# tensorflow/lingvo

Hardware: AMD Instinct MI355X
Metric: train step examples/sec (whole node), Librispeech Conformer-L (higher is better)
Workload: dtype bf16; 1 GPU; model=Conformer-L (17 blocks, d=512, h=8, kernel 32) + LSTM attention decoder, global_batch=512, seq_len=1200, parallelism=dp1, step_mode=hipgraph

## Files before the change

lingvo_amd/ops/hip/bindings.cpp:

```cpp
#include <torch/extension.h>

#include <vector>

std::vector<torch::Tensor> layer_norm_fwd(torch::Tensor x,
                                          torch::Tensor scale,
                                          torch::Tensor bias, double eps,
                                          bool rms);
std::vector<torch::Tensor> layer_norm_bwd(torch::Tensor dy, torch::Tensor x,
                                          torch::Tensor scale,
                                          torch::Tensor mean,
                                          torch::Tensor rstd, bool rms,
                                          c10::optional<torch::Tensor> dres);

torch::Tensor mfma_probe(torch::Tensor a, torch::Tensor bT);
torch::Tensor tr16_probe(torch::Tensor a, torch::Tensor b);

std::vector<torch::Tensor> fa_fwd(torch::Tensor q, torch::Tensor k,
                                  torch::Tensor v,
                                  c10::optional<torch::Tensor> klen,
                                  c10::optional<torch::Tensor> bias,
                                  c10::optional<torch::Tensor> qseg,
                                  c10::optional<torch::Tensor> kseg,
                                  int64_t win_l, int64_t win_r,
                                  int64_t bias_clip, double scale,
// ... 31 lines not shown
std::vector<torch::Tensor> glu_dwconv1d_bwd(
    torch::Tensor dy, torch::Tensor h, c10::optional<torch::Tensor> paddings,
    torch::Tensor w, int64_t pad, const std::string& route,
    c10::optional<torch::Tensor> dh_out, c10::optional<torch::Tensor> dw_out,
    c10::optional<torch::Tensor> db_out,
    c10::optional<torch::Tensor> dcol_out);

int64_t dwconv_tile_len();

std::vector<torch::Tensor> xent_fwd(torch::Tensor logits,
                                    torch::Tensor labels);
torch::Tensor xent_bwd(torch::Tensor logits, torch::Tensor labels,
                       torch::Tensor lse, torch::Tensor gout);

torch::Tensor dropout_fwd(torch::Tensor x, c10::optional<torch::Tensor> res,
                          int64_t seed,
                          c10::optional<torch::Tensor> step_seed,
                          double keep, int64_t act, double scale,
                          c10::optional<torch::Tensor> pad, int64_t d);
torch::Tensor dropout_bwd(torch::Tensor dy, c10::optional<torch::Tensor> x,
                          int64_t seed,
                          c10::optional<torch::Tensor> step_seed,
                          double keep, int64_t act, double scale,
                          c10::optional<torch::Tensor> pad, int64_t d);
std::vector<torch::Tensor> dropout_bwd_colsum(
    torch::Tensor dy, c10::optional<torch::Tensor> x, int64_t seed,
    c10::optional<torch::Tensor> step_seed, double keep, int64_t act,
    double scale, c10::optional<torch::Tensor> pad, int64_t d);

std::vector<torch::Tensor> group_norm_fwd(torch::Tensor x,
                                          torch::Tensor gamma,
                                          torch::Tensor beta,
                                          c10::optional<torch::Tensor> pad,
                                          int64_t groups, double eps,
                                          int64_t act,
                                          const std::string& route);
std::vector<torch::Tensor> group_norm_bwd(torch::Tensor dy, torch::Tensor x,
                                          torch::Tensor gamma,
                                          torch::Tensor beta,
                                          c10::optional<torch::Tensor> pad,
                                          torch::Tensor mean,
                                          torch::Tensor rstd,
                                          int64_t groups, int64_t act);

std::vector<torch::Tensor> lstm_gates_fwd_op(torch::Tensor gates,
                                             torch::Tensor c0, double fgb,
                                             double cap);
std::vector<torch::Tensor> lstm_gates_bwd_op(
    torch::Tensor gates, torch::Tensor c0, torch::Tensor c1,
    torch::Tensor dm1, c10::optional<torch::Tensor> dc1, double fgb,
    double cap);

void RegisterInputPipeline(py::module_& m);

void RegisterWpmTokenizer(py::module_& m);

void RegisterRecordBatcher(py::module_& m);

torch::Tensor emb_gather(torch::Tensor table, torch::Tensor ids,
                         double scale);
torch::Tensor emb_scatter_add(torch::Tensor dy, torch::Tensor ids,
                              int64_t vocab, double scale);

std::vector<torch::Tensor> moe_positions(torch::Tensor top1,
                                         torch::Tensor top2,
                                         int64_t num_experts);

torch::Tensor s2d_fwd(torch::Tensor x);
torch::Tensor s2d_inv(torch::Tensor dX, int64_t C);
torch::Tensor pad_scatter(torch::Tensor dout);

std::vector<torch::Tensor> topk_rows(torch::Tensor scores, int64_t k);

void smallm_gemm(torch::Tensor a, torch::Tensor wt,
                 c10::optional<torch::Tensor> pre, torch::Tensor out,
                 int64_t k, int64_t wt_col0, double alpha,
                 int64_t pre_mode);
std::vector<torch::Tensor> attend_fwd(torch::Tensor q, torch::Tensor enc,
                                      torch::Tensor pad, double scale);
std::vector<torch::Tensor> attend_bwd(torch::Tensor dctx,
                                      torch::Tensor probs, torch::Tensor q,
                                      torch::Tensor enc, torch::Tensor denc,
                                      double scale);
int64_t attend_lds_limit();
int64_t attend_lds_bytes(int64_t s, int64_t d, bool bwd);

void lstm_scan_fwd(torch::Tensor gates, torch::Tensor c, torch::Tensor m,
                   torch::Tensor pad, torch::Tensor wmt, int64_t rev_mask,
                   double fgb, double cap, int64_t s_begin, int64_t s_end,
                   int64_t rows_per_block);
void lstm_scan_bwd(torch::Tensor gates, torch::Tensor c, torch::Tensor pad,
                   torch::Tensor wm, c10::optional<torch::Tensor> dm_out,
                   c10::optional<torch::Tensor> dc_out,
                   torch::Tensor dgates, torch::Tensor dc_carry,
                   torch::Tensor dm_pass, int64_t rev_mask, double fgb,
                   double cap, int64_t s_begin, int64_t s_end,
                   int64_t rows_per_block);

std::vector<torch::Tensor> ctc_fwd(torch::Tensor logits,
                                   torch::Tensor logit_lengths,
                                   torch::Tensor labels,
                                   torch::Tensor label_lengths,
                                   int64_t blank);
torch::Tensor ctc_bwd(torch::Tensor logits, torch::Tensor logit_lengths,
                      torch::Tensor labels, torch::Tensor label_lengths,
                      torch::Tensor lse, torch::Tensor emis,
                      torch::Tensor alpha, torch::Tensor beta,
                      torch::Tensor nll, torch::Tensor valid,
                      torch::Tensor gout, int64_t blank);
int64_t ctc_max_label_len();

std::vector<torch::Tensor> rnnt_fwd(torch::Tensor logits,
                                    torch::Tensor logit_lengths,
                                    torch::Tensor labels,
                                    torch::Tensor label_lengths,
                                    int64_t blank);
torch::Tensor rnnt_bwd(torch::Tensor logits, torch::Tensor logit_lengths,
                       torch::Tensor labels, torch::Tensor label_lengths,
                       torch::Tensor lse, torch::Tensor emis,
                       torch::Tensor alpha, torch::Tensor beta,
                       torch::Tensor valid, torch::Tensor gnll,
                       int64_t blank);
int64_t rnnt_max_label_len();

torch::Tensor attn_decode(torch::Tensor q, torch::Tensor key_cache,
                          torch::Tensor value_cache,
                          c10::optional<torch::Tensor> q_start_t,
                          int64_t q_start,
                          c10::optional<torch::Tensor> bias, int64_t win_l,
                          int64_t bias_clip, double scale,
                          int64_t num_splits);
int64_t attn_decode_num_splits(int64_t B, int64_t NKV, int64_t keys,
                               int64_t rows);

PYBIND11_MODULE(TORCH_EXTENSION_NAME, m) {
  RegisterInputPipeline(m);
  RegisterWpmTokenizer(m);
  RegisterRecordBatcher(m);
  m.def("group_norm_fwd", &group_norm_fwd, "Fused padded GroupNorm fwd",
        py::arg("x"), py::arg("gamma"), py::arg("beta"), py::arg("pad"),
        py::arg("groups"), py::arg("eps"), py::arg("act"),
        py::arg("route") = "auto");
  m.def("group_norm_bwd", &group_norm_bwd, "Fused padded GroupNorm bwd");
  m.def("lstm_gates_fwd", &lstm_gates_fwd_op, "Fused LSTM gates fwd");
  m.def("lstm_gates_bwd", &lstm_gates_bwd_op, "Fused LSTM gates bwd");
  m.def("dropout_fwd", &dropout_fwd, "Fused dropout fwd");
  m.def("dropout_bwd", &dropout_bwd, "Fused dropout bwd");
  m.def("dropout_bwd_colsum", &dropout_bwd_colsum,
        "Fused dropout bwd + fp32 column sums of dx");
  m.def("xent_fwd", &xent_fwd, "Fused softmax-xent fwd");
  m.def("xent_bwd", &xent_bwd, "Fused softmax-xent bwd");
  m.def("dwconv1d_fwd", &dwconv1d_fwd, "Depthwise time conv fwd",
        py::arg("x"), py::arg("w"), py::arg("bias"), py::arg("pad"),
        py::arg("route") = "auto", py::arg("y_out") = py::none());
  m.def("dwconv1d_bwd", &dwconv1d_bwd, "Depthwise time conv bwd",
        py::arg("dy"), py::arg("x"), py::arg("w"), py::arg("pad"),
        py::arg("route") = "auto", py::arg("dx_out") = py::none(),
        py::arg("dw_out") = py::none(), py::arg("db_out") = py::none());
  m.def("glu_dwconv1d_fwd", &glu_dwconv1d_fwd,
        "conv(mask * glu(h)) + bias in one kernel", py::arg("h"),
        py::arg("paddings"), py::arg("w"), py::arg("bias"), py::arg("pad"),
        py::arg("route") = "auto", py::arg("y_out") = py::none());
  m.def("glu_dwconv1d_bwd", &glu_dwconv1d_bwd,
        "dh, dw, db and the fp32 column sums of dh of glu_dwconv1d_fwd",
        py::arg("dy"), py::arg("h"), py::arg("paddings"), py::arg("w"),
        py::arg("pad"), py::arg("route") = "auto",
        py::arg("dh_out") = py::none(), py::arg("dw_out") = py::none(),
        py::arg("db_out") = py::none(), py::arg("dcol_out") = py::none());
  m.def("dwconv_tile_len", &dwconv_tile_len,
        "Time rows per tile of the tiled depthwise convolution");
  m.def("layer_norm_fwd", &layer_norm_fwd, "Fused LayerNorm/RMSNorm fwd");
  m.def("layer_norm_bwd", &layer_norm_bwd, "Fused LayerNorm/RMSNorm bwd",
        py::arg("dy"), py::arg("x"), py::arg("scale"), py::arg("mean"),
        py::arg("rstd"), py::arg("rms"), py::arg("dres") = py::none());
  m.def("mfma_probe", &mfma_probe, "MFMA 16x16x32 layout probe");
  m.def("tr16_probe", &tr16_probe, "ds_read_tr16_b64 layout probe");
  m.def("fa_fwd", &fa_fwd, "Flash attention forward");
  m.def("fa_bwd", &fa_bwd, "Flash attention backward", py::arg("dout"),
        py::arg("q"), py::arg("k"), py::arg("v"), py::arg("o"),
        py::arg("lse"), py::arg("klen"), py::arg("bias"), py::arg("qseg"),
        py::arg("kseg"), py::arg("bias_grad"), py::arg("win_l"),
        py::arg("win_r"), py::arg("bias_clip"), py::arg("scale"),
        py::arg("chunk_size"), py::arg("left_chunks"),
        py::arg("dq_out") = py::none(), py::arg("dk_out") = py::none(),
        py::arg("dv_out") = py::none(), py::arg("route") = "auto");
  m.def("emb_gather", &emb_gather, "Embedding gather fwd");
  m.def("emb_scatter_add", &emb_scatter_add,
        "Deterministic embedding scatter-add bwd");
  m.def("moe_positions", &moe_positions,
        "Deterministic MoE top-2 position scan");
  m.def("smallm_gemm", &smallm_gemm,
        "Small-M MFMA GEMM (decode-step projections)");
  m.def("attend_fwd", &attend_fwd, "Fused dot-attention step fwd");
  m.def("attend_bwd", &attend_bwd, "Fused dot-attention step bwd");
  m.def("attend_lds_limit", &attend_lds_limit,
        "Dynamic LDS bytes an attend_* launch may ask for on this device");
  m.def("attend_lds_bytes", &attend_lds_bytes,
        "Dynamic LDS bytes attend_fwd/attend_bwd ask for at (S, D)");
  m.def("lstm_scan_fwd", &lstm_scan_fwd,
        "Fused LSTM scan forward: one launch per step, all directions");
  m.def("lstm_scan_bwd", &lstm_scan_bwd,
        "Fused LSTM scan backward: one launch per step, all directions");
  m.def("ctc_fwd", &ctc_fwd,
        "CTC loss forward: nll, valid and the backward's workspaces");
  m.def("ctc_bwd", &ctc_bwd, "CTC loss backward: dlogits");
  m.def("ctc_max_label_len", &ctc_max_label_len,
        "Largest label width L the CTC kernels support");
  m.def("rnnt_fwd", &rnnt_fwd,
        "Transducer loss forward: nll, valid and the backward's workspaces");
  m.def("rnnt_bwd", &rnnt_bwd, "Transducer loss backward: dlogits");
  m.def("rnnt_max_label_len", &rnnt_max_label_len,
        "Largest label width U the transducer kernels support");
  m.def("attn_decode", &attn_decode,
        "KV-cache attention (ExtendStep/StreamStep): split-K decode kernel "
        "+ combine",
        py::arg("q"), py::arg("key_cache"), py::arg("value_cache"),
        py::arg("q_start_t"), py::arg("q_start"), py::arg("bias"),
        py::arg("win_l"), py::arg("bias_clip"), py::arg("scale"),
        py::arg("num_splits") = 0);
  m.def("attn_decode_num_splits", &attn_decode_num_splits,
        "Split count attn_decode picks for (B, NKV, keys, rows = C * N/NKV)",
        py::arg("B"), py::arg("NKV"), py::arg("keys"), py::arg("rows") = 1);
  m.def("s2d_fwd", &s2d_fwd, "Space-to-depth + pad (conv frontend)");
  m.def("topk_rows", &topk_rows, "Row-wise top-k (beam pruning, K12)");
  m.def("s2d_inv", &s2d_inv, "Inverse space-to-depth");
  m.def("pad_scatter", &pad_scatter, "Zero-border pad scatter");
}
```

lingvo_amd/ops/hip/las_decoder.hip:

```cpp

#include <torch/extension.h>
#include <ATen/hip/HIPContext.h>

#include <atomic>

#include "common.h"
#include "mfma.h"

namespace {

__global__ __launch_bounds__(256) void smallm_gemm_kernel(
    const unsigned short* __restrict__ a, const unsigned short* __restrict__ wt,
    const unsigned short* __restrict__ pre, unsigned short* __restrict__ out,
    int m, int n, int k, long ldw, float alpha, int pre_mode) {
  const int nt = blockIdx.x;
  const int col0 = nt * 16;
  const int m0 = blockIdx.y * 128;
  const int wid = threadIdx.x / WAVE_SIZE;
  const int lane = threadIdx.x & 63;
  const int g = lane >> 4;
  const int cl = lane & 15;
  const int col = col0 + cl;
  const bool col_ok = col < n;

  constexpr int MT = 8;
  __shared__ float red[3][128][16];

  const int kq = (k / 32 + 3) / 4 * 32;
  const int k_lo = wid * kq;
  const int k_hi = min(k, k_lo + kq);

  f32x4 acc[MT];
#pragma unroll
  for (int mt = 0; mt < MT; ++mt) acc[mt] = {0.f, 0.f, 0.f, 0.f};

  for (int k0 = k_lo; k0 < k_hi; k0 += 32) {
    bf16x8 bf;
    if (col_ok) {
      bf = load_bf16x8_bits(wt + (long)col * ldw + k0 + g * 8);
    } else {
      float z[8] = {0, 0, 0, 0, 0, 0, 0, 0};
      bf = pack_bf16x8(z);
    }
#pragma unroll
    for (int mt = 0; mt < MT; ++mt) {
      const int row = m0 + mt * 16 + cl;
      bf16x8 af;
      if (row < m) {
        af = load_bf16x8_bits(a + (long)row * k + k0 + g * 8);
      } else {
        float z[8] = {0, 0, 0, 0, 0, 0, 0, 0};
        af = pack_bf16x8(z);
      }
      acc[mt] = mfma16x16x32_bf16(af, bf, acc[mt]);
    }
  }

  if (wid > 0) {
#pragma unroll
    for (int mt = 0; mt < MT; ++mt) {
#pragma unroll
      for (int r = 0; r < 4; ++r) {
        red[wid - 1][mt * 16 + g * 4 + r][cl] = acc[mt][r];
      }
    }
  }
  __syncthreads();
  if (wid != 0) return;
#pragma unroll
  for (int mt = 0; mt < MT; ++mt) {
#pragma unroll
    for (int r = 0; r < 4; ++r) {
      const int lrow = mt * 16 + g * 4 + r;
      const int row = m0 + lrow;
      if (row >= m || !col_ok) continue;
      float v = (acc[mt][r] + red[0][lrow][cl] + red[1][lrow][cl] +
                 red[2][lrow][cl]) * alpha;
      long off = (long)row * n + col;
      if (pre_mode == 1) {
        v += bf16_bits_to_float(pre[col]);
      } else if (pre_mode == 2) {
        v += bf16_bits_to_float(pre[off]);
      } else if (pre_mode == 3) {
        v += bf16_bits_to_float(out[off]);
      }
      out[off] = float_to_bf16_bits(v);
    }
// ... 196 lines not shown
        float t = wave_reduce_sum(part[u]);
        if (lane == 0) dl_s[s0 + u] = t;
      }
    }
  }
  __syncthreads();
  float t_part = 0.f;
  for (int s = threadIdx.x; s < s_len; s += 256) {
    t_part += pb[s] * dl_s[s];
  }
  t_part = wave_reduce_sum(t_part);
  if (lane == 0) red[wid] = t_part;
  __syncthreads();
  const float t = red[0] + red[1] + red[2] + red[3];

  __syncthreads();
  for (int s = threadIdx.x; s < s_len; s += 256) {
    dl_s[s] = pb[s] * (dl_s[s] - t) * scale;
  }
  __syncthreads();

  for (int i = threadIdx.x; i < 4 * d; i += 256) dq_s[i] = 0.f;
  __syncthreads();
  float* my_dq = dq_s + wid * d;
  float* db = denc + (long)b * s_len * d;
  for (int s0 = wid * 4; s0 < s_len; s0 += 16) {
    float dlv[4], ppv[4];
#pragma unroll
    for (int u = 0; u < 4; ++u) {
      dlv[u] = s0 + u < s_len ? dl_s[s0 + u] : 0.f;
      ppv[u] = s0 + u < s_len ? pb[s0 + u] : 0.f;
    }
    for (int v = 0; v < ndv; ++v) {
      const int i = lane * 8 + v * WAVE_SIZE * 8;
      if (i < d) {
        bf16x8 ev[4];
        floatx4 lo[4], hi[4];
#pragma unroll
        for (int u = 0; u < 4; ++u) {
          if (s0 + u < s_len) {
            ev[u] = load_bf16x8_bits(eb + (long)(s0 + u) * d + i);
            floatx4* dbv =
                reinterpret_cast<floatx4*>(db + (long)(s0 + u) * d + i);
            lo[u] = dbv[0];
            hi[u] = dbv[1];
          }
        }
        float dqacc[8] = {0, 0, 0, 0, 0, 0, 0, 0};
#pragma unroll
        for (int u = 0; u < 4; ++u) {
          if (s0 + u < s_len) {
#pragma unroll
            for (int j = 0; j < 4; ++j) {
              dqacc[j] += dlv[u] * (float)ev[u][j];
              lo[u][j] += dlv[u] * qreg[v][j] + ppv[u] * dcreg[v][j];
            }
#pragma unroll
            for (int j = 4; j < 8; ++j) {
              dqacc[j] += dlv[u] * (float)ev[u][j];
              hi[u][j - 4] += dlv[u] * qreg[v][j] + ppv[u] * dcreg[v][j];
            }
          }
        }
#pragma unroll
        for (int u = 0; u < 4; ++u) {
          if (s0 + u < s_len) {
            floatx4* dbv =
                reinterpret_cast<floatx4*>(db + (long)(s0 + u) * d + i);
            dbv[0] = lo[u];
            dbv[1] = hi[u];
          }
        }
#pragma unroll
        for (int j = 0; j < 8; ++j) {
          my_dq[i + j] += dqacc[j];
        }
      }
    }
  }
  __syncthreads();
  for (int i = threadIdx.x; i < d; i += 256) {
    dq[(long)b * d + i] = float_to_bf16_bits(
        dq_s[i] + dq_s[d + i] + dq_s[2 * d + i] + dq_s[3 * d + i]);
  }
}

}


namespace {

size_t lds_limit_bytes() {
  constexpr int kMaxDevices = 64;
  static std::atomic<int> cached[kMaxDevices];
  int dev = 0;
  LV_CHECK_HIP(hipGetDevice(&dev));
  const bool cacheable = dev >= 0 && dev < kMaxDevices;
  int limit = cacheable ? cached[dev].load(std::memory_order_relaxed) : 0;
  if (limit == 0) {
    LV_CHECK_HIP(hipDeviceGetAttribute(
        &limit, hipDeviceAttributeMaxSharedMemoryPerBlock, dev));
    if (cacheable) cached[dev].store(limit, std::memory_order_relaxed);
  }
  return (size_t)limit;
}

constexpr int64_t kAttendMaxD = 4 * WAVE_SIZE * 8;

size_t attend_fwd_lds(int64_t s, int64_t d) {
  return (size_t)d * 2 + (size_t)s * 4 + (size_t)4 * d * 4 + 16;
}

size_t attend_bwd_lds(int64_t s, int64_t d) {
  return (size_t)d * 4 + (size_t)s * 4 + (size_t)4 * d * 4 + 16;
}

bool cuda_contig(const torch::Tensor& t, torch::ScalarType st) {
  return t.is_cuda() && t.is_contiguous() && t.scalar_type() == st;
}

void check_attend_q_enc(const torch::Tensor& q, const torch::Tensor& enc) {
  TORCH_CHECK(cuda_contig(q, torch::kBFloat16) && q.dim() == 2,
              "q must be CUDA contiguous bf16 [B,D]");
  TORCH_CHECK(cuda_contig(enc, torch::kBFloat16) && enc.dim() == 3,
              "enc must be CUDA contiguous bf16 [B,S,D]");
  const int64_t b = q.size(0), d = q.size(1);
  TORCH_CHECK(b >= 1 && enc.size(0) == b && enc.size(2) == d,
              "enc must be [B,S,D] for q [B,D]");
  TORCH_CHECK(enc.size(1) >= 1, "S >= 1");
  TORCH_CHECK(d >= 8 && d % 8 == 0, "D % 8 == 0");
  TORCH_CHECK(d <= kAttendMaxD, "D <= 2048");
}

}

void smallm_gemm(torch::Tensor a, torch::Tensor wt,
                 c10::optional<torch::Tensor> pre, torch::Tensor out,
                 int64_t k, int64_t wt_col0, double alpha,
                 int64_t pre_mode) {
  TORCH_CHECK(cuda_contig(a, torch::kBFloat16) && a.dim() == 2,
              "a must be CUDA contiguous bf16 [M,K]");
  TORCH_CHECK(cuda_contig(wt, torch::kBFloat16) && wt.dim() == 2,
              "wt must be CUDA contiguous bf16 [>=N,ldw]");
  TORCH_CHECK(cuda_contig(out, torch::kBFloat16) && out.dim() == 2,
              "out must be CUDA contiguous bf16 [M,N]");
  TORCH_CHECK(out.size(0) == a.size(0), "out must have M rows");
  const int m = a.size(0);
  const int n = out.size(1);
  TORCH_CHECK(m >= 1 && n >= 1, "M, N >= 1");
  TORCH_CHECK(k >= 32 && k % 32 == 0, "K%32");
  TORCH_CHECK(k == a.size(1), "a must be [M,K] exactly");

  TORCH_CHECK(wt.size(0) >= n, "wt rows >= N");
  const long ldw = wt.size(1);
  TORCH_CHECK(wt_col0 >= 0 && wt_col0 + k <= ldw, "wt K slice OOB");
  TORCH_CHECK(ldw % 8 == 0 && wt_col0 % 8 == 0,
              "ldw % 8 == 0 and wt_col0 % 8 == 0");
  TORCH_CHECK(pre_mode >= 0 && pre_mode <= 3, "pre_mode in 0..3");
  const unsigned short* prep = nullptr;
  if (pre_mode == 1 || pre_mode == 2) {
    TORCH_CHECK(pre.has_value() && cuda_contig(*pre, torch::kBFloat16),
                "pre must be CUDA contiguous bf16");
    if (pre_mode == 1) {
      TORCH_CHECK(pre->numel() == n, "mode 1: pre must have N elements");
    } else {
      TORCH_CHECK(pre->dim() == 2 && pre->size(0) == m && pre->size(1) == n,
                  "mode 2: pre must be [M,N]");
    }
    prep = (const unsigned short*)pre->data_ptr();
  }
  auto stream = at::cuda::getCurrentCUDAStream();
  hipLaunchKernelGGL(smallm_gemm_kernel,
                     dim3(cdiv(n, 16), cdiv(m, 128)), dim3(256), 0,
                     stream, (const unsigned short*)a.data_ptr(),
                     (const unsigned short*)wt.data_ptr() + wt_col0,
                     prep, (unsigned short*)out.data_ptr(), m, n, (int)k,
                     ldw, (float)alpha, (int)pre_mode);
  LV_CHECK_HIP(hipGetLastError());
}

std::vector<torch::Tensor> attend_fwd(torch::Tensor q, torch::Tensor enc,
                                      torch::Tensor pad, double scale) {
  check_attend_q_enc(q, enc);
  const int b = q.size(0), d = q.size(1);
  const int s = enc.size(1);
  TORCH_CHECK(cuda_contig(pad, torch::kFloat32) && pad.dim() == 2 &&
              pad.size(0) == b && pad.size(1) == s,
              "pad must be CUDA contiguous fp32 [B,S]");
  const size_t shmem = attend_fwd_lds(s, d);
  TORCH_CHECK(shmem <= lds_limit_bytes(), "attend_fwd: S=", s, " D=", d,
              " needs ", shmem, " bytes of LDS, over the device limit");
  auto probs = torch::empty({b, s}, q.options().dtype(torch::kFloat32));
  auto ctx = torch::empty({b, d}, q.options());
  auto stream = at::cuda::getCurrentCUDAStream();
  hipLaunchKernelGGL(attend_fwd_kernel, dim3(b), dim3(256), shmem, stream,
                     (const unsigned short*)q.data_ptr(),
                     (const unsigned short*)enc.data_ptr(),
                     pad.data_ptr<float>(), probs.data_ptr<float>(),
                     (unsigned short*)ctx.data_ptr(), b, s, d,
                     (float)scale);
  LV_CHECK_HIP(hipGetLastError());
  return {probs, ctx};
}

std::vector<torch::Tensor> attend_bwd(torch::Tensor dctx,
                                      torch::Tensor probs, torch::Tensor q,
                                      torch::Tensor enc, torch::Tensor denc,
                                      double scale) {
  check_attend_q_enc(q, enc);
  const int b = q.size(0), d = q.size(1);
  const int s = enc.size(1);
  TORCH_CHECK(dctx.is_cuda() && dctx.is_floating_point() &&
              dctx.dim() == 2 && dctx.size(0) == b && dctx.size(1) == d,
              "dctx must be a CUDA float tensor [B,D]");
  TORCH_CHECK(cuda_contig(probs, torch::kFloat32) && probs.dim() == 2 &&
              probs.size(0) == b && probs.size(1) == s,
              "probs must be CUDA contiguous fp32 [B,S]");
  TORCH_CHECK(cuda_contig(denc, torch::kFloat32) && denc.dim() == 3 &&
              denc.size(0) == b && denc.size(1) == s && denc.size(2) == d,
              "denc must be CUDA contiguous fp32 [B,S,D]");
  const size_t shmem = attend_bwd_lds(s, d);
  TORCH_CHECK(shmem <= lds_limit_bytes(), "attend_bwd: S=", s, " D=", d,
              " needs ", shmem, " bytes of LDS, over the device limit");
  auto dctx_c = dctx.to(torch::kBFloat16).contiguous();
  auto dq = torch::empty({b, d}, q.options());
  auto stream = at::cuda::getCurrentCUDAStream();
  hipLaunchKernelGGL(attend_bwd_kernel, dim3(b), dim3(256), shmem, stream,
                     (const unsigned short*)dctx_c.data_ptr(),
                     probs.data_ptr<float>(),
                     (const unsigned short*)q.data_ptr(),
                     (const unsigned short*)enc.data_ptr(),
                     (unsigned short*)dq.data_ptr(),
                     denc.data_ptr<float>(), b, s, d, (float)scale);
  LV_CHECK_HIP(hipGetLastError());
  return {dq};
}

int64_t attend_lds_limit() { return (int64_t)lds_limit_bytes(); }

int64_t attend_lds_bytes(int64_t s, int64_t d, bool bwd) {
  return (int64_t)(bwd ? attend_bwd_lds(s, d) : attend_fwd_lds(s, d));
}
```

lingvo_amd/ops/las_decoder.py:

```python

from __future__ import annotations

import math
from typing import Optional

import torch

from lingvo_amd.ops import _loader


class _DecoderRecurrenceFn(torch.autograd.Function):

  @staticmethod
  def forward(ctx, emb_gates, w_cm0, b1, wm1, wq, enc, enc_pad, fgb, cap,
              src_dim):
    ext = _loader.get_ext(required=True)
    B, L, G4 = emb_gates.shape
    H = G4 // 4
    D = wq.shape[1]
    scale = 1.0 / math.sqrt(D)
    dt = torch.bfloat16
    emb_gates_b = emb_gates.to(dt).contiguous()
    enc_b = enc.to(dt).contiguous()
    pad_f = enc_pad.float().contiguous()
    w1t = w_cm0.t().contiguous().to(dt)
    wm1t = wm1.t().contiguous().to(dt)
    wqt = wq.t().contiguous().to(dt)
    b1_b = b1.to(dt).contiguous()

    dev = enc.device
    gates0 = torch.empty(L, B, G4, dtype=dt, device=dev)
    gates1 = torch.empty(L, B, G4, dtype=dt, device=dev)
    qs = torch.empty(L, B, D, dtype=dt, device=dev)
    eg_t = emb_gates_b.permute(1, 0, 2).contiguous()
    c0s, m0s, c1s, m1s, ctxs, probs_l = [], [], [], [], [], []
    zeros_h = torch.zeros(B, H, dtype=dt, device=dev)
    c0, m0, c1, m1 = zeros_h, zeros_h, zeros_h, zeros_h
    ctxv = torch.zeros(B, D, dtype=dt, device=dev)
    for t in range(L):
      g0 = gates0[t]
      ext.smallm_gemm(ctxv, w1t, eg_t[t], g0, src_dim, 0, 1.0, 2)
      ext.smallm_gemm(m0, w1t, None, g0, H, src_dim, 1.0, 3)
      c0, m0 = ext.lstm_gates_fwd(g0, c0, fgb, cap)
      g1 = gates1[t]
      ext.smallm_gemm(m0, wm1t, b1_b, g1, H, 0, 1.0, 1)
      ext.smallm_gemm(m1, wm1t, None, g1, H, H, 1.0, 3)
      c1, m1 = ext.lstm_gates_fwd(g1, c1, fgb, cap)
      q = qs[t]
      ext.smallm_gemm(m1, wqt, None, q, H, 0, 1.0, 0)
      p, ctxv = ext.attend_fwd(q, enc_b, pad_f, scale)
      c0s.append(c0)
      m0s.append(m0)
      c1s.append(c1)
      m1s.append(m1)
      ctxs.append(ctxv)
      probs_l.append(p)

    m1_st = torch.stack(m1s)
    ctx_st = torch.stack(ctxs)
    ctx.save_for_backward(
        emb_gates_b, w_cm0, wm1, wq, enc_b, pad_f, gates0, gates1, qs,
        torch.stack(c0s), torch.stack(m0s), torch.stack(c1s), m1_st,
        ctx_st, torch.stack(probs_l))
    ctx.cfg = (fgb, cap, src_dim, scale, b1.dtype, enc.dtype,
               emb_gates.dtype)
    out = torch.cat(
        [m1_st.permute(1, 0, 2), ctx_st.permute(1, 0, 2)], dim=-1)
    return out

  @staticmethod
  def backward(ctx, dout):
    ext = _loader.get_ext(required=True)
    (emb_gates_b, w_cm0, wm1, wq, enc_b, pad_f, gates0, gates1, qs, c0s,
     m0s, c1s, m1s, ctxs, probs) = ctx.saved_tensors
    fgb, cap, src_dim, scale, b1_dtype, enc_dtype, eg_dtype = ctx.cfg
    L, B, G4 = gates0.shape
    H = G4 // 4
    D = qs.shape[-1]
    dt = torch.bfloat16
    dev = dout.device
    dout = dout.to(dt)
    w_cm0_b = w_cm0.to(dt).contiguous()
    wm1_b = wm1.to(dt).contiguous()
    wq_b = wq.to(dt).contiguous()

    denc = torch.zeros(B, enc_b.shape[1], D, dtype=torch.float32,
                       device=dev)
    dgates0 = torch.empty(L, B, G4, dtype=dt, device=dev)
    dgates1 = torch.empty(L, B, G4, dtype=dt, device=dev)
    dqs = torch.empty(L, B, D, dtype=dt, device=dev)
    zeros_h = torch.zeros(B, H, dtype=dt, device=dev)
    dctx_carry = torch.zeros(B, D, dtype=dt, device=dev)
    dm0_carry = zeros_h
    dm1_carry = zeros_h
    dc0_carry: Optional[torch.Tensor] = None
    dc1_carry: Optional[torch.Tensor] = None
    dmm = torch.empty(B, 2 * H, dtype=dt, device=dev)
    dcm = torch.empty(B, src_dim + H, dtype=dt, device=dev)
    dm1_total = torch.empty(B, H, dtype=dt, device=dev)
    dout_t = dout.permute(1, 0, 2)
    dm1_parts = dout_t[:, :, :H].contiguous()
    dctx_parts = dout_t[:, :, H:].contiguous()
    for t in range(L - 1, -1, -1):
      dctx_total = dctx_parts[t] + dctx_carry
      dq = ext.attend_bwd(dctx_total, probs[t], qs[t], enc_b, denc,
                          scale)[0]
      dqs[t] = dq
      pre_m1 = dm1_parts[t] + dm1_carry
      ext.smallm_gemm(dq, wq_b, pre_m1, dm1_total, D, 0, 1.0, 2)
      c1_prev = c1s[t - 1] if t > 0 else zeros_h
      dg1, dc1_carry = ext.lstm_gates_bwd(
          gates1[t], c1_prev, c1s[t], dm1_total, dc1_carry, fgb, cap)
      dgates1[t] = dg1
      ext.smallm_gemm(dg1, wm1_b, None, dmm, G4, 0, 1.0, 0)
      dm0_total = (dmm[:, :H] + dm0_carry).contiguous()
      c0_prev = c0s[t - 1] if t > 0 else zeros_h
      dg0, dc0_carry = ext.lstm_gates_bwd(
          gates0[t], c0_prev, c0s[t], dm0_total, dc0_carry, fgb, cap)
      dgates0[t] = dg0
      ext.smallm_gemm(dg0, w_cm0_b, None, dcm, G4, 0, 1.0, 0)
      dctx_carry = dcm[:, :src_dim].contiguous()
      dm0_carry = dcm[:, src_dim:].contiguous()
      dm1_carry = dmm[:, H:].contiguous()

    ctx_prev = torch.cat(
        [torch.zeros(1, B, D, dtype=dt, device=dev), ctxs[:-1]])
    m0_prev = torch.cat(
        [torch.zeros(1, B, H, dtype=dt, device=dev), m0s[:-1]])
    m1_prev = torch.cat(
        [torch.zeros(1, B, H, dtype=dt, device=dev), m1s[:-1]])
    x0 = torch.cat([ctx_prev, m0_prev], dim=-1).reshape(L * B, -1)
    dw_cm0 = (x0.t() @ dgates0.reshape(L * B, G4)).to(w_cm0.dtype)
    x1 = torch.cat([m0s, m1_prev], dim=-1).reshape(L * B, -1)
    dwm1 = (x1.t() @ dgates1.reshape(L * B, G4)).to(wm1.dtype)
    db1 = dgates1.float().sum(dim=(0, 1)).to(b1_dtype)
    dwq = (m1s.reshape(L * B, H).t() @ dqs.reshape(L * B, D)).to(wq.dtype)
    demb_gates = dgates0.permute(1, 0, 2).to(eg_dtype)
    return (demb_gates, dw_cm0, db1, dwm1, dwq, denc.to(enc_dtype),
            None, None, None, None)


def decoder_recurrence(emb_gates: torch.Tensor, w_cm0: torch.Tensor,
                       b1: torch.Tensor, wm1: torch.Tensor,
                       wq: torch.Tensor, enc: torch.Tensor,
                       enc_pad: torch.Tensor, fgb: float, cap: float,
                       src_dim: int) -> torch.Tensor:
  return _DecoderRecurrenceFn.apply(emb_gates, w_cm0, b1, wm1, wq, enc,
                                    enc_pad, fgb, cap, src_dim)
```

Measured before the change: 1399 examples/sec.

## Defer decoder attention dEnc to one batched kernel after the recurrence

Adds one-pass attention step kernels. The forward writes probs, ctx and an fp32 ctx into preallocated stacked buffers. The backward now emits only dctx, dlogits and dq per step and no longer accumulates dEnc into a [B,S,D] fp32 buffer at every decoder step. The encoder gradient is then computed once after the loop by a tiled kernel that sums over all steps, as dl·q + p·dctx. This removes the per-step read-modify-write of the full dEnc tensor, at the cost of storing per-step dl, dctx and ctx32 stacks. It is enabled by default through the 'auto' route.

```diff
diff --git a/lingvo_amd/ops/hip/bindings.cpp b/lingvo_amd/ops/hip/bindings.cpp
--- a/lingvo_amd/ops/hip/bindings.cpp
+++ b/lingvo_amd/ops/hip/bindings.cpp
@@ -137,6 +137,18 @@
                                       torch::Tensor probs, torch::Tensor q,
                                       torch::Tensor enc, torch::Tensor denc,
                                       double scale);
+void attend_step_fwd(torch::Tensor q, torch::Tensor enc, torch::Tensor pad,
+                     double scale, torch::Tensor probs, torch::Tensor ctx,
+                     torch::Tensor ctx32, int64_t variant);
+void attend_step_bwd(torch::Tensor dctx_a, c10::optional<torch::Tensor> dctx_b,
+                     torch::Tensor probs, torch::Tensor ctx32,
+                     torch::Tensor enc, double scale, torch::Tensor dctx_out,
+                     torch::Tensor dl, torch::Tensor dq, int64_t variant);
+void attend_denc(torch::Tensor dl, torch::Tensor probs, torch::Tensor qs,
+                 torch::Tensor dctx, torch::Tensor out);
+int64_t attend_step_lds_bytes(int64_t s, int64_t d, bool bwd,
+                              int64_t variant);
+int64_t attend_denc_row_tile();
 int64_t attend_lds_limit();
 int64_t attend_lds_bytes(int64_t s, int64_t d, bool bwd);
 
@@ -248,6 +260,23 @@
         "Small-M MFMA GEMM (decode-step projections)");
   m.def("attend_fwd", &attend_fwd, "Fused dot-attention step fwd");
   m.def("attend_bwd", &attend_bwd, "Fused dot-attention step bwd");
+  m.def("attend_step_fwd", &attend_step_fwd,
+        "One-pass dot-attention step fwd into caller rows (probs, ctx, ctx32)",
+        py::arg("q"), py::arg("enc"), py::arg("pad"), py::arg("scale"),
+        py::arg("probs"), py::arg("ctx"), py::arg("ctx32"),
+        py::arg("variant") = 0);
+  m.def("attend_step_bwd", &attend_step_bwd,
+        "One-pass dot-attention step bwd without dEnc (dctx, dl, dq out)",
+        py::arg("dctx_a"), py::arg("dctx_b"), py::arg("probs"),
+        py::arg("ctx32"), py::arg("enc"), py::arg("scale"),
+        py::arg("dctx_out"), py::arg("dl"), py::arg("dq"),
+        py::arg("variant") = 0);
+  m.def("attend_denc", &attend_denc,
+        "dEnc of the whole recurrence from the stacked dl, probs, q, dctx");
+  m.def("attend_step_lds_bytes", &attend_step_lds_bytes,
+        "Dynamic LDS bytes attend_step_fwd/bwd ask for at (S, D, variant)");
+  m.def("attend_denc_row_tile", &attend_denc_row_tile,
+        "Rows of S one attend_denc workgroup owns");
   m.def("attend_lds_limit", &attend_lds_limit,
         "Dynamic LDS bytes an attend_* launch may ask for on this device");
   m.def("attend_lds_bytes", &attend_lds_bytes,
diff --git a/lingvo_amd/ops/hip/las_decoder.hip b/lingvo_amd/ops/hip/las_decoder.hip
--- a/lingvo_amd/ops/hip/las_decoder.hip
+++ b/lingvo_amd/ops/hip/las_decoder.hip
@@ -3,6 +3,7 @@
 #include <ATen/hip/HIPContext.h>
 
 #include <atomic>
+#include <climits>
 
 #include "common.h"
 #include "mfma.h"
@@ -365,6 +366,312 @@
   for (int i = threadIdx.x; i < d; i += 256) {
     dq[(long)b * d + i] = float_to_bf16_bits(
         dq_s[i] + dq_s[d + i] + dq_s[2 * d + i] + dq_s[3 * d + i]);
+  }
+}
+
+
+
+template <int NDV, int U>
+__device__ __forceinline__ void load_enc_rows(
+    const unsigned short* __restrict__ eb, int s0, int s_len, int d, int lane,
+    bf16x8 (&ev)[U][NDV]) {
+  const float z[8] = {0, 0, 0, 0, 0, 0, 0, 0};
+  const bf16x8 zero = pack_bf16x8(z);
+#pragma unroll
+  for (int u = 0; u < U; ++u) {
+#pragma unroll
+    for (int v = 0; v < NDV; ++v) {
+      const int i = lane * 8 + v * WAVE_SIZE * 8;
+      ev[u][v] = (s0 + u < s_len && i < d)
+                     ? load_bf16x8_bits(eb + (long)(s0 + u) * d + i)
+                     : zero;
+    }
+  }
+}
+
+template <int NDV, int U, int NW>
+__global__ __launch_bounds__(NW * WAVE_SIZE) void attend_step_fwd_kernel(
+    const unsigned short* __restrict__ q, const unsigned short* __restrict__ enc,
+    const float* __restrict__ pad, float* __restrict__ probs,
+    unsigned short* __restrict__ ctx, float* __restrict__ ctx32, int s_len,
+    int d, float scale) {
+  constexpr int NT = NW * WAVE_SIZE;
+  const int b = blockIdx.x;
+  const int wid = threadIdx.x / WAVE_SIZE;
+  const int lane = threadIdx.x & 63;
+  extern __shared__ char smem[];
+  float* logit_s = (float*)smem;
+  float* ctx_s = logit_s + s_len;
+  float* red = ctx_s + NW * d;
+
+  float qreg[NDV][8];
+#pragma unroll
+  for (int v = 0; v < NDV; ++v) {
+    const int i = lane * 8 + v * WAVE_SIZE * 8;
+    if (i < d) {
+      bf16x8 qv = load_bf16x8_bits(q + (long)b * d + i);
+#pragma unroll
+      for (int j = 0; j < 8; ++j) qreg[v][j] = (float)qv[j];
+    } else {
+#pragma unroll
+      for (int j = 0; j < 8; ++j) qreg[v][j] = 0.f;
+    }
+  }
+
+  const unsigned short* eb = enc + (long)b * s_len * d;
+  const float* padb = pad + (long)b * s_len;
+  float m = -1e30f;
+  float acc[NDV][8];
+#pragma unroll
+  for (int v = 0; v < NDV; ++v) {
+#pragma unroll
+    for (int j = 0; j < 8; ++j) acc[v][j] = 0.f;
+  }
+  for (int s0 = wid * U; s0 < s_len; s0 += NW * U) {
+    bf16x8 ev[U][NDV];
+    load_enc_rows<NDV, U>(eb, s0, s_len, d, lane, ev);
+    float mask[U];
+#pragma unroll
+    for (int u = 0; u < U; ++u) {
+      mask[u] = (s0 + u >= s_len || padb[s0 + u] > 0.5f) ? -1e30f : 0.f;
+    }
+    float lg[U];
+    float mnew = m;
+#pragma unroll
+    for (int u = 0; u < U; ++u) {
+      float part = 0.f;
+#pragma unroll
+      for (int v = 0; v < NDV; ++v) {
+#pragma unroll
+        for (int j = 0; j < 8; ++j) part += qreg[v][j] * (float)ev[u][v][j];
+      }
+      lg[u] = wave_reduce_sum(part) * scale + mask[u];
+      if (s0 + u < s_len) {
+        mnew = fmaxf(mnew, lg[u]);
+        if (lane == 0) logit_s[s0 + u] = lg[u];
+      }
+    }
+    const float f = __expf(m - mnew);
+    m = mnew;
+#pragma unroll
+    for (int v = 0; v < NDV; ++v) {
+#pragma unroll
+      for (int j = 0; j < 8; ++j) acc[v][j] *= f;
+    }
+#pragma unroll
+    for (int u = 0; u < U; ++u) {
+      const float p = __expf(lg[u] - mnew);
+#pragma unroll
+      for (int v = 0; v < NDV; ++v) {
+#pragma unroll
+        for (int j = 0; j < 8; ++j) acc[v][j] += p * (float)ev[u][v][j];
+      }
+    }
+  }
+  if (lane == 0) red[wid] = m;
+  __syncthreads();
+  float lmax = red[0];
+#pragma unroll
+  for (int w = 1; w < NW; ++w) lmax = fmaxf(lmax, red[w]);
+  {
+    const float wgt = __expf(m - lmax);
+#pragma unroll
+    for (int v = 0; v < NDV; ++v) {
+      const int i = lane * 8 + v * WAVE_SIZE * 8;
+      if (i < d) {
+#pragma unroll
+        for (int j = 0; j < 8; ++j) ctx_s[wid * d + i + j] = acc[v][j] * wgt;
+      }
+    }
+  }
+  float lsum = 0.f;
+  for (int s = threadIdx.x; s < s_len; s += NT) {
+    float e = __expf(logit_s[s] - lmax);
+    logit_s[s] = e;
+    lsum += e;
+  }
+  lsum = wave_reduce_sum(lsum);
+  __syncthreads();
+  if (lane == 0) red[wid] = lsum;
+  __syncthreads();
+  lsum = 0.f;
+#pragma unroll
+  for (int w = 0; w < NW; ++w) lsum += red[w];
+  const float inv = lsum > 0.f ? 1.f / lsum : 0.f;
+  for (int s = threadIdx.x; s < s_len; s += NT) {
+    probs[(long)b * s_len + s] = logit_s[s] * inv;
+  }
+  for (int i = threadIdx.x; i < d; i += NT) {
+    float c = 0.f;
+#pragma unroll
+    for (int w = 0; w < NW; ++w) c += ctx_s[w * d + i];
+    c *= inv;
+    ctx32[(long)b * d + i] = c;
+    ctx[(long)b * d + i] = float_to_bf16_bits(c);
+  }
+}
+
+template <int NDV, int U, int NW>
+__global__ __launch_bounds__(NW * WAVE_SIZE) void attend_step_bwd_kernel(
+    const unsigned short* __restrict__ dctx_a,
+    const unsigned short* __restrict__ dctx_b, long ldb,
+    const float* __restrict__ probs, const float* __restrict__ ctx32,
+    const unsigned short* __restrict__ enc,
+    unsigned short* __restrict__ dctx_out, float* __restrict__ dl_out,
+    unsigned short* __restrict__ dq, int s_len, int d, float scale) {
+  constexpr int NT = NW * WAVE_SIZE;
+  const int b = blockIdx.x;
+  const int wid = threadIdx.x / WAVE_SIZE;
+  const int lane = threadIdx.x & 63;
+  extern __shared__ char smem[];
+  float* dc_s = (float*)smem;
+  float* dq_s = dc_s + d;
+  float* red = dq_s + NW * d;
+
+  float t_part = 0.f;
+  for (int i = threadIdx.x; i < d; i += NT) {
+    unsigned short bits = dctx_a[(long)b * d + i];
+    if (dctx_b != nullptr) {
+      bits = float_to_bf16_bits(bf16_bits_to_float(bits) +
+                                bf16_bits_to_float(dctx_b[(long)b * ldb + i]));
+    }
+    dctx_out[(long)b * d + i] = bits;
+    const float v = bf16_bits_to_float(bits);
+    dc_s[i] = v;
+    t_part += v * ctx32[(long)b * d + i];
+  }
+  const float t = block_reduce_sum<NW>(t_part, red);
+
+  float dcreg[NDV][8];
+#pragma unroll
+  for (int v = 0; v < NDV; ++v) {
+    const int i = lane * 8 + v * WAVE_SIZE * 8;
+#pragma unroll
+    for (int j = 0; j < 8; ++j) dcreg[v][j] = i < d ? dc_s[i + j] : 0.f;
+  }
+
+  const unsigned short* eb = enc + (long)b * s_len * d;
+  const float* pb = probs + (long)b * s_len;
+  float* dlb = dl_out + (long)b * s_len;
+  float acc[NDV][8];
+#pragma unroll
+  for (int v = 0; v < NDV; ++v) {
+#pragma unroll
+    for (int j = 0; j < 8; ++j) acc[v][j] = 0.f;
+  }
+  for (int s0 = wid * U; s0 < s_len; s0 += NW * U) {
+    bf16x8 ev[U][NDV];
+    load_enc_rows<NDV, U>(eb, s0, s_len, d, lane, ev);
+    float pv[U];
+#pragma unroll
+    for (int u = 0; u < U; ++u) pv[u] = s0 + u < s_len ? pb[s0 + u] : 0.f;
+#pragma unroll
+    for (int u = 0; u < U; ++u) {
+      float part = 0.f;
+#pragma unroll
+      for (int v = 0; v < NDV; ++v) {
+#pragma unroll
+        for (int j = 0; j < 8; ++j) part += dcreg[v][j] * (float)ev[u][v][j];
+      }
+      const float dlv = pv[u] * (wave_reduce_sum(part) - t) * scale;
+      if (lane == u && s0 + u < s_len) dlb[s0 + u] = dlv;
+#pragma unroll
+      for (int v = 0; v < NDV; ++v) {
+#pragma unroll
+        for (int j = 0; j < 8; ++j) acc[v][j] += dlv * (float)ev[u][v][j];
+      }
+    }
+  }
+#pragma unroll
+  for (int v = 0; v < NDV; ++v) {
+    const int i = lane * 8 + v * WAVE_SIZE * 8;
+    if (i < d) {
+#pragma unroll
+      for (int j = 0; j < 8; ++j) dq_s[wid * d + i + j] = acc[v][j];
+    }
+  }
+  __syncthreads();
+  for (int i = threadIdx.x; i < d; i += NT) {
+    float c = 0.f;
+#pragma unroll
+    for (int w = 0; w < NW; ++w) c += dq_s[w * d + i];
+    dq[(long)b * d + i] = float_to_bf16_bits(c);
+  }
+}
+
+constexpr int kDencRows = 8;
+constexpr int kDencTile = 4 * kDencRows;
+constexpr int kDencSteps = 64;
+
+__device__ __forceinline__ void store_denc(float* p, const float* a) {
+  floatx4* pv = reinterpret_cast<floatx4*>(p);
+  pv[0] = floatx4{a[0], a[1], a[2], a[3]};
+  pv[1] = floatx4{a[4], a[5], a[6], a[7]};
+}
+
+__device__ __forceinline__ void store_denc(unsigned short* p, const float* a) {
+  ushortx8 o;
+#pragma unroll
+  for (int j = 0; j < 8; ++j) o[j] = float_to_bf16_bits(a[j]);
+  *reinterpret_cast<ushortx8*>(p) = o;
+}
+
+template <typename OutT>
+__global__ __launch_bounds__(256) void attend_denc_kernel(
+    const float* __restrict__ dl, const float* __restrict__ probs,
+    const unsigned short* __restrict__ qs,
+    const unsigned short* __restrict__ dctx, OutT* __restrict__ out,
+    int l_total, int b_total, int s_len, int d, int s_tiles) {
+  const int b = blockIdx.x / s_tiles;
+  const int s_base = (blockIdx.x % s_tiles) * kDencTile;
+  const int wid = threadIdx.x / WAVE_SIZE;
+  const int lane = threadIdx.x & 63;
+  const int c0 = blockIdx.y * WAVE_SIZE * 8 + lane * 8;
+  __shared__ float sc[kDencSteps][kDencTile][2];
+
+  float acc[kDencRows][8];
+#pragma unroll
+  for (int r = 0; r < kDencRows; ++r) {
+#pragma unroll
+    for (int j = 0; j < 8; ++j) acc[r][j] = 0.f;
+  }
+  for (int l0 = 0; l0 < l_total; l0 += kDencSteps) {
+    __syncthreads();
+    for (int idx = threadIdx.x; idx < kDencSteps * kDencTile; idx += 256) {
+      const int ll = idx / kDencTile, r = idx % kDencTile;
+      const int l = l0 + ll, s = s_base + r;
+      const bool ok = l < l_total && s < s_len;
+      const long off = ((long)l * b_total + b) * s_len + s;
+      sc[ll][r][0] = ok ? dl[off] : 0.f;
+      sc[ll][r][1] = ok ? probs[off] : 0.f;
+    }
+    __syncthreads();
+    if (c0 < d) {
+      const int l_cnt = min(kDencSteps, l_total - l0);
+#pragma unroll 4
+      for (int ll = 0; ll < l_cnt; ++ll) {
+        const long off = ((long)(l0 + ll) * b_total + b) * d + c0;
+        const bf16x8 qv = load_bf16x8_bits(qs + off);
+        const bf16x8 dv = load_bf16x8_bits(dctx + off);
+#pragma unroll
+        for (int r = 0; r < kDencRows; ++r) {
+          const float a = sc[ll][wid * kDencRows + r][0];
+          const float p = sc[ll][wid * kDencRows + r][1];
+#pragma unroll
+          for (int j = 0; j < 8; ++j) {
+            acc[r][j] += a * (float)qv[j];
+            acc[r][j] += p * (float)dv[j];
+          }
+        }
+      }
+    }
+  }
+  if (c0 < d) {
+#pragma unroll
+    for (int r = 0; r < kDencRows; ++r) {
+      const int s = s_base + wid * kDencRows + r;
+      if (s < s_len) store_denc(out + ((long)b * s_len + s) * d + c0, acc[r]);
+    }
   }
 }
 
@@ -524,3 +831,188 @@
 int64_t attend_lds_bytes(int64_t s, int64_t d, bool bwd) {
   return (int64_t)(bwd ? attend_bwd_lds(s, d) : attend_fwd_lds(s, d));
 }
+
+
+namespace {
+
+bool step_variant(int64_t variant, int64_t d, int* u, int* nw) {
+  if (variant == 0) variant = d <= 2 * WAVE_SIZE * 8 ? 3 : 1;
+  if (variant < 1 || variant > 4) return false;
+  *u = (variant == 2 || variant == 4) ? 8 : 4;
+  *nw = variant >= 3 ? 8 : 4;
+  return *u == 4 || d <= 2 * WAVE_SIZE * 8;
+}
+
+size_t attend_step_fwd_lds(int64_t s, int64_t d, int nw) {
+  return (size_t)s * 4 + (size_t)nw * d * 4 + (size_t)nw * 4;
+}
+
+size_t attend_step_bwd_lds(int64_t s, int64_t d, int nw) {
+  (void)s;
+  return (size_t)d * 4 + (size_t)nw * d * 4 + (size_t)nw * 4;
+}
+
+bool cuda_rows(const torch::Tensor& t, torch::ScalarType st, int64_t rows,
+               int64_t cols) {
+  return t.is_cuda() && t.scalar_type() == st && t.dim() == 2 &&
+         t.size(0) == rows && t.size(1) == cols && t.is_contiguous();
+}
+
+#define LV_STEP_CASE(NDV, U, NW, KERNEL, ...)                               \
+  if (ndv == NDV && u == U && nw == NW) {                                   \
+    hipLaunchKernelGGL((KERNEL<NDV, U, NW>), dim3(b), dim3(NW * WAVE_SIZE), \
+                       shmem, stream, __VA_ARGS__);                         \
+  } else
+
+#define LV_STEP_NDV(NDV, KERNEL, ...)         \
+  LV_STEP_CASE(NDV, 4, 4, KERNEL, __VA_ARGS__) \
+  LV_STEP_CASE(NDV, 8, 4, KERNEL, __VA_ARGS__) \
+  LV_STEP_CASE(NDV, 4, 8, KERNEL, __VA_ARGS__) \
+  LV_STEP_CASE(NDV, 8, 8, KERNEL, __VA_ARGS__)
+
+#define LV_STEP_DISPATCH(KERNEL, ...)                          \
+  LV_STEP_NDV(1, KERNEL, __VA_ARGS__)                          \
+  LV_STEP_NDV(2, KERNEL, __VA_ARGS__)                          \
+  LV_STEP_CASE(3, 4, 4, KERNEL, __VA_ARGS__)                   \
+  LV_STEP_CASE(3, 4, 8, KERNEL, __VA_ARGS__)                   \
+  LV_STEP_CASE(4, 4, 4, KERNEL, __VA_ARGS__)                   \
+  LV_STEP_CASE(4, 4, 8, KERNEL, __VA_ARGS__) {                 \
+    TORCH_CHECK(false, "no kernel for ndv=", ndv, " u=", u, " nw=", nw); \
+  }
+
+}
+
+void attend_step_fwd(torch::Tensor q, torch::Tensor enc, torch::Tensor pad,
+                     double scale, torch::Tensor probs, torch::Tensor ctx,
+                     torch::Tensor ctx32, int64_t variant) {
+  check_attend_q_enc(q, enc);
+  const int b = q.size(0), d = q.size(1);
+  const int s = enc.size(1);
+  TORCH_CHECK(cuda_contig(pad, torch::kFloat32) && pad.dim() == 2 &&
+              pad.size(0) == b && pad.size(1) == s,
+              "pad must be CUDA contiguous fp32 [B,S]");
+  TORCH_CHECK(cuda_rows(probs, torch::kFloat32, b, s),
+              "probs must be CUDA contiguous fp32 [B,S]");
+  TORCH_CHECK(cuda_rows(ctx, torch::kBFloat16, b, d),
+              "ctx must be CUDA contiguous bf16 [B,D]");
+  TORCH_CHECK(cuda_rows(ctx32, torch::kFloat32, b, d),
+              "ctx32 must be CUDA contiguous fp32 [B,D]");
+  int u = 0, nw = 0;
+  TORCH_CHECK(step_variant(variant, d, &u, &nw),
+              "variant in 0..4, and 2 or 4 only for D <= 1024");
+  const size_t shmem = attend_step_fwd_lds(s, d, nw);
+  TORCH_CHECK(shmem <= lds_limit_bytes(), "attend_step_fwd: S=", s, " D=", d,
+              " needs ", shmem, " bytes of LDS, over the device limit");
+  const int ndv = cdiv(d, WAVE_SIZE * 8);
+  auto stream = at::cuda::getCurrentCUDAStream();
+  LV_STEP_DISPATCH(attend_step_fwd_kernel,
+                   (const unsigned short*)q.data_ptr(),
+                   (const unsigned short*)enc.data_ptr(),
+                   pad.data_ptr<float>(), probs.data_ptr<float>(),
+                   (unsigned short*)ctx.data_ptr(), ctx32.data_ptr<float>(),
+                   s, d, (float)scale)
+  LV_CHECK_HIP(hipGetLastError());
+}
+
+void attend_step_bwd(torch::Tensor dctx_a, c10::optional<torch::Tensor> dctx_b,
+                     torch::Tensor probs, torch::Tensor ctx32,
+                     torch::Tensor enc, double scale, torch::Tensor dctx_out,
+                     torch::Tensor dl, torch::Tensor dq, int64_t variant) {
+  check_attend_q_enc(dctx_a, enc);
+  const int b = dctx_a.size(0), d = dctx_a.size(1);
+  const int s = enc.size(1);
+  const unsigned short* bp = nullptr;
+  long ldb = 0;
+  if (dctx_b.has_value()) {
+    const torch::Tensor& t = *dctx_b;
+    TORCH_CHECK(t.is_cuda() && t.scalar_type() == torch::kBFloat16 &&
+                t.dim() == 2 && t.size(0) == b && t.size(1) == d &&
+                t.stride(1) == 1 && t.stride(0) >= d,
+                "dctx_b must be CUDA bf16 [B,D] with unit column stride");
+    bp = (const unsigned short*)t.data_ptr();
+    ldb = t.stride(0);
+  }
+  TORCH_CHECK(cuda_rows(probs, torch::kFloat32, b, s),
+              "probs must be CUDA contiguous fp32 [B,S]");
+  TORCH_CHECK(cuda_rows(ctx32, torch::kFloat32, b, d),
+              "ctx32 must be CUDA contiguous fp32 [B,D]");
+  TORCH_CHECK(cuda_rows(dctx_out, torch::kBFloat16, b, d),
+              "dctx_out must be CUDA contiguous bf16 [B,D]");
+  TORCH_CHECK(cuda_rows(dl, torch::kFloat32, b, s),
+              "dl must be CUDA contiguous fp32 [B,S]");
+  TORCH_CHECK(cuda_rows(dq, torch::kBFloat16, b, d),
+              "dq must be CUDA contiguous bf16 [B,D]");
+  int u = 0, nw = 0;
+  TORCH_CHECK(step_variant(variant, d, &u, &nw),
+              "variant in 0..4, and 2 or 4 only for D <= 1024");
+  const size_t shmem = attend_step_bwd_lds(s, d, nw);
+  TORCH_CHECK(shmem <= lds_limit_bytes(), "attend_step_bwd: S=", s, " D=", d,
+              " needs ", shmem, " bytes of LDS, over the device limit");
+  const int ndv = cdiv(d, WAVE_SIZE * 8);
+  auto stream = at::cuda::getCurrentCUDAStream();
+  LV_STEP_DISPATCH(attend_step_bwd_kernel,
+                   (const unsigned short*)dctx_a.data_ptr(), bp, ldb,
+                   probs.data_ptr<float>(), ctx32.data_ptr<float>(),
+                   (const unsigned short*)enc.data_ptr(),
+                   (unsigned short*)dctx_out.data_ptr(),
+                   dl.data_ptr<float>(), (unsigned short*)dq.data_ptr(), s,
+                   d, (float)scale)
+  LV_CHECK_HIP(hipGetLastError());
+}
+
+void attend_denc(torch::Tensor dl, torch::Tensor probs, torch::Tensor qs,
+                 torch::Tensor dctx, torch::Tensor out) {
+  TORCH_CHECK(cuda_contig(dl, torch::kFloat32) && dl.dim() == 3,
+              "dl must be CUDA contiguous fp32 [L,B,S]");
+  const int64_t l = dl.size(0), b = dl.size(1), s = dl.size(2);
+  TORCH_CHECK(l >= 1 && b >= 1 && s >= 1, "L, B, S >= 1");
+  TORCH_CHECK(cuda_contig(probs, torch::kFloat32) &&
+              probs.sizes() == dl.sizes(),
+              "probs must be CUDA contiguous fp32 [L,B,S]");
+  TORCH_CHECK(cuda_contig(qs, torch::kBFloat16) && qs.dim() == 3 &&
+              qs.size(0) == l && qs.size(1) == b,
+              "qs must be CUDA contiguous bf16 [L,B,D]");
+  const int64_t d = qs.size(2);
+  TORCH_CHECK(d >= 8 && d % 8 == 0, "D % 8 == 0");
+  TORCH_CHECK(d <= kAttendMaxD, "D <= 2048");
+  TORCH_CHECK(cuda_contig(dctx, torch::kBFloat16) &&
+              dctx.sizes() == qs.sizes(),
+              "dctx must be CUDA contiguous bf16 [L,B,D]");
+  TORCH_CHECK(out.is_cuda() && out.is_contiguous() && out.dim() == 3 &&
+              out.size(0) == b && out.size(1) == s && out.size(2) == d &&
+              (out.scalar_type() == torch::kFloat32 ||
+               out.scalar_type() == torch::kBFloat16),
+              "out must be CUDA contiguous fp32 or bf16 [B,S,D]");
+  TORCH_CHECK(l <= INT_MAX && b <= INT_MAX && s <= INT_MAX, "sizes fit int");
+  const int64_t s_tiles = (s + kDencTile - 1) / kDencTile;
+  TORCH_CHECK(b * s_tiles <= INT_MAX, "B * ceil(S/32) fits the grid");
+  const dim3 grid((unsigned)(b * s_tiles), cdiv(d, WAVE_SIZE * 8));
+  auto stream = at::cuda::getCurrentCUDAStream();
+  if (out.scalar_type() == torch::kFloat32) {
+    hipLaunchKernelGGL(attend_denc_kernel<float>, grid, dim3(256), 0, stream,
+                       dl.data_ptr<float>(), probs.data_ptr<float>(),
+                       (const unsigned short*)qs.data_ptr(),
+                       (const unsigned short*)dctx.data_ptr(),
+                       out.data_ptr<float>(), (int)l, (int)b, (int)s, (int)d,
+                       (int)s_tiles);
+  } else {
+    hipLaunchKernelGGL(attend_denc_kernel<unsigned short>, grid, dim3(256), 0,
+                       stream, dl.data_ptr<float>(), probs.data_ptr<float>(),
+                       (const unsigned short*)qs.data_ptr(),
+                       (const unsigned short*)dctx.data_ptr(),
+                       (unsigned short*)out.data_ptr(), (int)l, (int)b,
+                       (int)s, (int)d, (int)s_tiles);
+  }
+  LV_CHECK_HIP(hipGetLastError());
+}
+
+int64_t attend_step_lds_bytes(int64_t s, int64_t d, bool bwd,
+                              int64_t variant) {
+  int u = 0, nw = 0;
+  TORCH_CHECK(step_variant(variant, d, &u, &nw),
+              "variant in 0..4, and 2 or 4 only for D <= 1024");
+  return (int64_t)(bwd ? attend_step_bwd_lds(s, d, nw)
+                       : attend_step_fwd_lds(s, d, nw));
+}
+
+int64_t attend_denc_row_tile() { return kDencTile; }
diff --git a/lingvo_amd/ops/las_decoder.py b/lingvo_amd/ops/las_decoder.py
--- a/lingvo_amd/ops/las_decoder.py
+++ b/lingvo_amd/ops/las_decoder.py
@@ -13,7 +13,7 @@
 
   @staticmethod
   def forward(ctx, emb_gates, w_cm0, b1, wm1, wq, enc, enc_pad, fgb, cap,
-              src_dim):
+              src_dim, deferred):
     ext = _loader.get_ext(required=True)
     B, L, G4 = emb_gates.shape
     H = G4 // 4
@@ -37,6 +37,11 @@
     zeros_h = torch.zeros(B, H, dtype=dt, device=dev)
     c0, m0, c1, m1 = zeros_h, zeros_h, zeros_h, zeros_h
     ctxv = torch.zeros(B, D, dtype=dt, device=dev)
+    if deferred:
+      S = enc_b.shape[1]
+      ctx_st = torch.empty(L, B, D, dtype=dt, device=dev)
+      ctx32_st = torch.empty(L, B, D, dtype=torch.float32, device=dev)
+      probs_st = torch.empty(L, B, S, dtype=torch.float32, device=dev)
     for t in range(L):
       g0 = gates0[t]
       ext.smallm_gemm(ctxv, w1t, eg_t[t], g0, src_dim, 0, 1.0, 2)
@@ -48,22 +53,30 @@
       c1, m1 = ext.lstm_gates_fwd(g1, c1, fgb, cap)
       q = qs[t]
       ext.smallm_gemm(m1, wqt, None, q, H, 0, 1.0, 0)
-      p, ctxv = ext.attend_fwd(q, enc_b, pad_f, scale)
+      if deferred:
+        ctxv = ctx_st[t]
+        ext.attend_step_fwd(q, enc_b, pad_f, scale, probs_st[t], ctxv,
+                            ctx32_st[t])
+      else:
+        p, ctxv = ext.attend_fwd(q, enc_b, pad_f, scale)
+        ctxs.append(ctxv)
+        probs_l.append(p)
       c0s.append(c0)
       m0s.append(m0)
       c1s.append(c1)
       m1s.append(m1)
-      ctxs.append(ctxv)
-      probs_l.append(p)
 
     m1_st = torch.stack(m1s)
-    ctx_st = torch.stack(ctxs)
+    if not deferred:
+      ctx_st = torch.stack(ctxs)
+      probs_st = torch.stack(probs_l)
+      ctx32_st = torch.empty(0, device=dev)
     ctx.save_for_backward(
         emb_gates_b, w_cm0, wm1, wq, enc_b, pad_f, gates0, gates1, qs,
         torch.stack(c0s), torch.stack(m0s), torch.stack(c1s), m1_st,
-        ctx_st, torch.stack(probs_l))
+        ctx_st, probs_st, ctx32_st)
     ctx.cfg = (fgb, cap, src_dim, scale, b1.dtype, enc.dtype,
-               emb_gates.dtype)
+               emb_gates.dtype, deferred)
     out = torch.cat(
         [m1_st.permute(1, 0, 2), ctx_st.permute(1, 0, 2)], dim=-1)
     return out
@@ -72,8 +85,9 @@
   def backward(ctx, dout):
     ext = _loader.get_ext(required=True)
     (emb_gates_b, w_cm0, wm1, wq, enc_b, pad_f, gates0, gates1, qs, c0s,
-     m0s, c1s, m1s, ctxs, probs) = ctx.saved_tensors
-    fgb, cap, src_dim, scale, b1_dtype, enc_dtype, eg_dtype = ctx.cfg
+     m0s, c1s, m1s, ctxs, probs, ctx32s) = ctx.saved_tensors
+    (fgb, cap, src_dim, scale, b1_dtype, enc_dtype, eg_dtype,
+     deferred) = ctx.cfg
     L, B, G4 = gates0.shape
     H = G4 // 4
     D = qs.shape[-1]
@@ -84,13 +98,18 @@
     wm1_b = wm1.to(dt).contiguous()
     wq_b = wq.to(dt).contiguous()
 
-    denc = torch.zeros(B, enc_b.shape[1], D, dtype=torch.float32,
-                       device=dev)
+    S = enc_b.shape[1]
+    if deferred:
+      dctx_st = torch.empty(L, B, D, dtype=dt, device=dev)
+      dl_st = torch.empty(L, B, S, dtype=torch.float32, device=dev)
+    else:
+      denc = torch.zeros(B, S, D, dtype=torch.float32, device=dev)
     dgates0 = torch.empty(L, B, G4, dtype=dt, device=dev)
     dgates1 = torch.empty(L, B, G4, dtype=dt, device=dev)
     dqs = torch.empty(L, B, D, dtype=dt, device=dev)
     zeros_h = torch.zeros(B, H, dtype=dt, device=dev)
-    dctx_carry = torch.zeros(B, D, dtype=dt, device=dev)
+    dctx_carry = None if deferred else \
+        torch.zeros(B, D, dtype=dt, device=dev)
     dm0_carry = zeros_h
     dm1_carry = zeros_h
     dc0_carry: Optional[torch.Tensor] = None
@@ -102,10 +121,15 @@
     dm1_parts = dout_t[:, :, :H].contiguous()
     dctx_parts = dout_t[:, :, H:].contiguous()
     for t in range(L - 1, -1, -1):
-      dctx_total = dctx_parts[t] + dctx_carry
-      dq = ext.attend_bwd(dctx_total, probs[t], qs[t], enc_b, denc,
-                          scale)[0]
-      dqs[t] = dq
+      if deferred:
+        dq = dqs[t]
+        ext.attend_step_bwd(dctx_parts[t], dctx_carry, probs[t], ctx32s[t],
+                            enc_b, scale, dctx_st[t], dl_st[t], dq)
+      else:
+        dctx_total = dctx_parts[t] + dctx_carry
+        dq = ext.attend_bwd(dctx_total, probs[t], qs[t], enc_b, denc,
+                            scale)[0]
+        dqs[t] = dq
       pre_m1 = dm1_parts[t] + dm1_carry
       ext.smallm_gemm(dq, wq_b, pre_m1, dm1_total, D, 0, 1.0, 2)
       c1_prev = c1s[t - 1] if t > 0 else zeros_h
@@ -119,7 +143,9 @@
           gates0[t], c0_prev, c0s[t], dm0_total, dc0_carry, fgb, cap)
       dgates0[t] = dg0
       ext.smallm_gemm(dg0, w_cm0_b, None, dcm, G4, 0, 1.0, 0)
-      dctx_carry = dcm[:, :src_dim].contiguous()
+      dctx_carry = dcm[:, :src_dim]
+      if not deferred:
+        dctx_carry = dctx_carry.contiguous()
       dm0_carry = dcm[:, src_dim:].contiguous()
       dm1_carry = dmm[:, H:].contiguous()
 
@@ -136,14 +162,23 @@
     db1 = dgates1.float().sum(dim=(0, 1)).to(b1_dtype)
     dwq = (m1s.reshape(L * B, H).t() @ dqs.reshape(L * B, D)).to(wq.dtype)
     demb_gates = dgates0.permute(1, 0, 2).to(eg_dtype)
+    if deferred:
+      denc = torch.empty(
+          B, S, D, device=dev,
+          dtype=dt if enc_dtype == torch.bfloat16 else torch.float32)
+      ext.attend_denc(dl_st, probs, qs, dctx_st, denc)
     return (demb_gates, dw_cm0, db1, dwm1, dwq, denc.to(enc_dtype),
-            None, None, None, None)
+            None, None, None, None, None)
 
 
 def decoder_recurrence(emb_gates: torch.Tensor, w_cm0: torch.Tensor,
                        b1: torch.Tensor, wm1: torch.Tensor,
                        wq: torch.Tensor, enc: torch.Tensor,
                        enc_pad: torch.Tensor, fgb: float, cap: float,
-                       src_dim: int) -> torch.Tensor:
+                       src_dim: int,
+                       attend_route: str = 'auto') -> torch.Tensor:
+  if attend_route not in ('auto', 'deferred', 'accumulate'):
+    raise ValueError(f'unknown attend_route {attend_route!r}')
   return _DecoderRecurrenceFn.apply(emb_gates, w_cm0, b1, wm1, wq, enc,
-                                    enc_pad, fgb, cap, src_dim)
+                                    enc_pad, fgb, cap, src_dim,
+                                    attend_route != 'accumulate')
```

After: 1456 examples/sec (median of 6 runs). 1.04x the previous value.
